# tmdt-buw/VQ-VAE-Transformer-Arc-Welding

Measured on AMD Instinct MI355X. Metric: welding windows/sec (train) VQ-VAE+8-blk Transformer at 1/2/4/8 MI355X, higher is better.
Workload: dtype bf16; 1 GPU; VQ-VAE-Patch reconstruction train step (configs[1]); global_batch=1024, per_gpu_batch=1024, seq_len=200, codebook=512x64, hidden=512, n_resblocks=8, patch=25, parallelism=dp1, optimizer=RAdam(lr 1e-3), operands=bf16 (opt-in), fp32 accumulation and master weights

## Files before the change

### include/arcweld_amd.h

```cpp
#ifndef ARCWELD_AMD_H
#define ARCWELD_AMD_H

#include <stdint.h>

#ifdef __cplusplus
extern "C" {
#endif

enum { AW_OK = 0, AW_ERR_ARG = -1, AW_ERR_LAUNCH = -2 };
enum { AW_F32 = 0, AW_BF16 = 1 };
enum { AW_ACT_GELU_ERF = 0, AW_ACT_GELU_TANH = 1, AW_ACT_DERIV = 2 };

const char* aw_last_error(void);
int aw_version(void);

typedef struct {
  int M, N, K;
  int a_dtype;
  const void* A; int64_t lda; int a_trans;
  const void* B; int64_t ldb; int b_trans;
  int conv_cin, conv_seg, conv_dir, conv_operand;
  float alpha, beta;
  const float* bias;
  int act;
// ... 62 lines not shown
  int head_k;
  const void* head_in;
  const void* head_w;
  const float* head_bias;
  void* head_patches;
  int head_L, head_C, head_P;
} aw_res_chain_fwd_args;
typedef struct {
  int64_t N;
  int H, R;
  int taps, seg;
  const void* gx;
  const void* gxo;
  const void* x0;
  const void* w1t[AW_RES_CHAIN_MAX];
  const void* w2t[AW_RES_CHAIN_MAX];
  const void* dgelu_h[AW_RES_CHAIN_MAX];
  const void* dgelu_x[AW_RES_CHAIN_MAX];
  void* gh[AW_RES_CHAIN_MAX];
  void* gxo_out[AW_RES_CHAIN_MAX];
  float drop_p;
  int store_policy;
  const uint64_t* drop_masks;
} aw_res_chain_bwd_args;
int aw_res_chain_fwd(const aw_res_chain_fwd_args* args, void* stream);
int aw_res_chain_bwd(const aw_res_chain_bwd_args* args, void* stream);
int64_t aw_res_dropout_masks_bytes(int64_t N, int R);
int aw_res_dropout_masks(int64_t N, int R, float drop_p, const uint64_t* drop_seed, const uint64_t* seed_ptr,
                         void* masks, void* stream);
#define AW_RES_PACK_MAX 32
int aw_res_pack_weights(const void* const* src, void* const* fwd, void* const* bwd, int n, int taps, void* stream);
int aw_res_pack_weights_mixed(const void* const* src, void* const* fwd, void* const* bwd, const int* job_taps, int n,
                              int taps, void* stream);

int aw_vq_forward(const float* z, const float* E, int64_t N, int K, int D,
                  float* zq, int64_t* idx, float* counts, double* sqerr, void* stream);
int aw_vq_forward_ex(const float* z, const float* E, int64_t N, int K, int D, float* zq, int64_t* idx, float* counts,
                     double* sqerr, void* zq_copy, int copy_dtype, void* stream);
#define AW_VQ_COUNT_GROUPS_MAX 64
int aw_vq_forward_ex2(const float* z, const float* E, int64_t N, int K, int D, float* zq, int64_t* idx, float* counts,
                      int count_groups, double* sqerr, void* zq_copy, int copy_dtype, void* stream);
int aw_vq_finalize(const float* counts, const double* sqerr, int64_t N, int K, int D, float beta,
                   float* loss, float* perplexity, void* stream);
int aw_vq_finalize_ex(const float* counts, int count_groups, const double* sqerr, int64_t N, int K, int D, float beta,
                      float* loss, float* perplexity, void* stream);
int aw_vq_backward(const float* z, const float* E, const int64_t* idx, const float* g_zq, const float* g_loss,
// ... 208 lines not shown
```

### vq-vae-transformer-arc-welding_amd/arcweld/_native.py

```python
from __future__ import annotations

import ctypes
import os

import torch

PKG_DIR = os.path.dirname(os.path.dirname(os.path.abspath(__file__)))
LIB_PATH = os.environ.get("ARCWELD_LIB") or os.path.join(PKG_DIR, "lib", "libarcweld_amd.so")
HEADER = os.path.join(os.path.dirname(PKG_DIR), "include", "arcweld_amd.h")

AW_F32, AW_BF16 = 0, 1
AW_ACT_GELU_ERF, AW_ACT_GELU_TANH, AW_ACT_DERIV = 0, 1, 2
AW_STORE_NT, AW_STORE_WT = 0, 1

c_i64 = ctypes.c_int64
c_int = ctypes.c_int
c_f = ctypes.c_float
c_p = ctypes.c_void_p


class GemmArgs(ctypes.Structure):
    _fields_ = [
        ("M", c_int), ("N", c_int), ("K", c_int),
        ("a_dtype", c_int),
# ... 36 lines not shown
RES_PACK_MAX = 32
RES_TAIL_MAX = 8
SAMPLE_MAX_V = 16384
_E = RES_CHAIN_MAX


class ResChainFwdArgs(ctypes.Structure):
    _fields_ = [("N", c_i64), ("H", c_int), ("R", c_int), ("taps", c_int), ("seg", c_int), ("a0", c_p), ("x0", c_p),
                ("w1", c_p * _E), ("w2", c_p * _E), ("b1", c_p * _E), ("b2", c_p * _E),
                ("dgelu_h", c_p * _E), ("a1", c_p * _E), ("dgelu_x", c_p * _E), ("a", c_p * _E),
                ("drop_p", c_f), ("drop_seed", ctypes.c_uint64 * _E), ("seed_ptr", c_p), ("store_policy", c_int),
                ("drop_masks", c_p),
                ("tail_k1", c_int), ("tail_w", c_p * RES_TAIL_MAX), ("tail_bias", c_p), ("tail_y", c_p),
                ("tail_colstats", c_p),
                ("sep_d", c_int), ("sep_w", c_p), ("sep_bias", c_p), ("sep_z", c_p),
                ("head_k", c_int), ("head_in", c_p), ("head_w", c_p), ("head_bias", c_p), ("head_patches", c_p),
                ("head_L", c_int), ("head_C", c_int), ("head_P", c_int)]


class ResChainBwdArgs(ctypes.Structure):
    _fields_ = [("N", c_i64), ("H", c_int), ("R", c_int), ("taps", c_int), ("seg", c_int), ("gx", c_p), ("gxo", c_p),
                ("x0", c_p), ("w1t", c_p * _E), ("w2t", c_p * _E), ("dgelu_h", c_p * _E), ("dgelu_x", c_p * _E),
                ("gh", c_p * _E), ("gxo_out", c_p * _E),
                ("drop_p", c_f), ("store_policy", c_int), ("drop_masks", c_p)]


class SampleArgs(ctypes.Structure):
    _fields_ = [("logits", c_p), ("B", c_int), ("V", c_int), ("n_valid", c_int),
                ("top_k", c_int), ("top_p", c_f), ("min_p", c_f), ("inv_temperature", c_f),
                ("do_sample", c_int), ("seed", ctypes.c_uint64), ("step", c_i64),
                ("ids_out", c_p), ("ld_ids", c_i64), ("col", c_i64),
                ("u_out", c_p),
                ("logp_out", c_p), ("logq_out", c_p), ("ld_lp", c_i64), ("col_lp", c_i64),
                ("n_kept_out", c_p), ("thr_out", c_p),
                ("bad_count", c_p)]


BEAM_MAX_W = 32


class BeamArgs(ctypes.Structure):
    _fields_ = [("logits", c_p), ("ldl", c_i64), ("B", c_int), ("W_in", c_int), ("W_out", c_int), ("V", c_int),
                ("n_valid", c_int),
                ("scores_in", c_p),
                ("scores_out", c_p), ("parent_out", c_p), ("token_out", c_p), ("logp_out", c_p),
                ("bad_count", c_p)]

# ... 181 lines not shown
```

### vq-vae-transformer-arc-welding_amd/arcweld/kernels.py

```python
from __future__ import annotations

import contextvars
import ctypes

import torch

from . import _native as nat
from ._native import AW_ACT_DERIV, AW_ACT_GELU_ERF, AW_ACT_GELU_TANH, AW_BF16, AW_F32, GemmArgs, call, dtype_code, ptr, stream_ptr

__all__ = ["gemm", "AW_ACT_DERIV", "AW_ACT_GELU_ERF", "AW_ACT_GELU_TANH", "AW_BF16", "AW_F32"]


def _ld(t):
    if t is None:
        return 0
    if t.dim() == 1:
        return t.shape[0]
    if t.stride(-1) != 1:
        raise nat.NativeError("operand rows must be contiguous (stride(-1) == 1)")
    return t.stride(0)


_STORE_POLICY = contextvars.ContextVar("arcweld_store_policy", default=0)

# ... 309 lines not shown
            hp = None
        else:
            hp, P = head[3], int(head[4])
            if hin.dtype != torch.float32 or hin.dim() != 3 or not hin.is_contiguous():
                raise nat.NativeError("res_chain_fwd: the encoder head's input must be contiguous (B, L, C) float32 windows")
            Bw, Lw, Cw = hin.shape
            if not (1 <= P <= hk) or (Lw * Cw) % P or Bw * (Lw * Cw // P) != N:
                raise nat.NativeError(f"res_chain_fwd: windows {tuple(hin.shape)} do not make {N} patches of {P}")
            if hp is not None and (hp.dtype != torch.bfloat16 or tuple(hp.shape) != (N, hk) or not hp.is_contiguous()):
                raise nat.NativeError(f"res_chain_fwd: patches must be a contiguous ({N}, {hk}) bfloat16 tensor")
            g.head_patches, g.head_L, g.head_C, g.head_P = ptr(hp), Lw, Cw, P
        g.head_k, g.head_in, g.head_w, g.head_bias = hk, ptr(hin), ptr(hw), ptr(hb)
        flops += 2.0 * N * H * (hk if taps == 3 else P)
        extra += [hin, hw, hb, hp]
    elif a0 is None or x0 is None:
        raise nat.NativeError("res_chain_fwd: a0 / x0 missing")
    _maybe_timed(stream, "gemm_bf16", flops,
                 lambda sp: call("aw_res_chain_fwd", ctypes.byref(g), sp),
                 lambda: (f"res_chain_fwd_kernel<{int(taps)}>",
                          _nbytes([a0, x0, masks] + list(w1) + list(w2) + list(b1) + list(b2) + list(dh) + list(a1) +
                                  list(dx)[:-1] + list(a) + extra)))


def res_chain_bwd(gx, gxo, w1t, w2t, dh, x0, dx, gh, gxo_out, drop_p=0.0, masks=None, taps=1, seg=16, stream=None):
    N, H = gx.shape
    R = len(w1t)
    if not (1 <= R <= RES_CHAIN_MAX) or not all(len(v) == R for v in (w2t, dh, dx, gh, gxo_out)):
        raise nat.NativeError("res_chain_bwd: need R (1..16) entries in every per-block list")
    _chk_rows([gx, gxo, x0] + list(dh) + list(dx[1:]) + list(gh) + list(gxo_out), N, H, "res_chain_bwd")
    g = nat.ResChainBwdArgs()
    g.N, g.H, g.R, g.taps, g.seg = N, H, R, int(taps), int(seg)
    g.gx, g.gxo, g.x0 = ptr(gx), ptr(gxo), ptr(x0)
    for r in range(R):
        g.w1t[r], g.w2t[r], g.dgelu_h[r] = ptr(w1t[r]), ptr(w2t[r]), ptr(dh[r])
        g.dgelu_x[r] = ptr(dx[r]) if r > 0 else None
        g.gh[r], g.gxo_out[r] = ptr(gh[r]), ptr(gxo_out[r])
    g.drop_p = float(drop_p)
    g.store_policy = _chain_store_policy()
    g.drop_masks = ptr(masks)
    _maybe_timed(stream, "gemm_bf16", _chain_flops(R, N, H, taps, seg),
                 lambda sp: call("aw_res_chain_bwd", ctypes.byref(g), sp),
                 lambda: (f"res_chain_bwd_kernel<{int(taps)}>",
                          _nbytes([gx, gxo, x0, masks] + list(w1t) + list(w2t) + list(dh) + list(dx[1:]) + list(gh) +
                                  list(gxo_out))))


def res_pack_weights(src, fwd=None, bwd=None, taps=1, stream=None, job_taps=None):
    n = len(src)
    fwd = fwd if fwd is not None else [None] * n
    bwd = bwd if bwd is not None else [None] * n
    jt = [int(taps)] * n if job_taps is None else [int(v) for v in job_taps]
    if len(fwd) != n or len(bwd) != n or len(jt) != n:
        raise nat.NativeError("res_pack_weights: list lengths differ")
    for i in range(n):
        for t in (src[i], fwd[i], bwd[i]):
            if t is not None and (t.dtype != torch.bfloat16 or t.numel() != 512 * 512 * jt[i] or not t.is_contiguous()):
                raise nat.NativeError(f"res_pack_weights: need contiguous 512 x {512 * jt[i]} bfloat16 tensors")
    for c0 in range(0, n, nat.RES_PACK_MAX):
        sl = slice(c0, c0 + nat.RES_PACK_MAX)
        m = len(src[sl])
        arr = lambda ts: (ctypes.c_void_p * m)(*[ptr(t) for t in ts])
        if job_taps is None:
            call("aw_res_pack_weights", arr(src[sl]), arr(fwd[sl]), arr(bwd[sl]), m, int(taps), stream_ptr(stream))
        else:
            call("aw_res_pack_weights_mixed", arr(src[sl]), arr(fwd[sl]), arr(bwd[sl]), (ctypes.c_int * m)(*jt[sl]), m,
                 int(taps), stream_ptr(stream))

# ... 659 lines not shown
```

### vq-vae-transformer-arc-welding_amd/arcweld/resstack.py

```python
from __future__ import annotations

import torch

from . import kernels as K

F32 = torch.float32


def _centre_job(w, out):
    O, I = w.shape[0], w.shape[1]
    c = w[:, :, 1]
    if w.is_contiguous():
        return (w, O, I, 3, 1, 0, out)
    if not c.is_contiguous():
        raise ValueError("encoder conv weight: unsupported layout")
    return (c, O, I, 1, 0, 0, out)


def _centre_grad(g):
    O, I = g.shape[0], g.shape[1]
    if g.is_contiguous():
        return g.view(O, 3 * I), (0, 3, 1)
    c = g[:, :, 1]
    if not c.is_contiguous():
# ... 117 lines not shown
    sv.xs += [e(RT) if save and r < R - 1 else None for r in range(R)]
    sv.a0s += [e(T) for _ in range(R)]
    wsrc = [w for r in range(R) for w in weights[r]]
    pk = [torch.empty(H, geo.Kd, device=dev, dtype=T) for _ in wsrc]
    ktail = None
    if tail is not None:
        Wt, tb, Y, cst = tail
        k1 = Wt.shape[0] // H
        tsrc = [Wt[j * H:(j + 1) * H] for j in range(k1)]
        tpk = [torch.empty(H, H, device=dev, dtype=T) for _ in tsrc]
        K.res_pack_weights(wsrc + tsrc, pk + tpk, None, taps=taps, job_taps=[taps] * len(wsrc) + [1] * k1)
        ktail = (tpk, tb, Y, cst)
    else:
        K.res_pack_weights(wsrc, pk, None, taps=taps)
    if save:
        sv.pk_bwd = wsrc
        if sv.p_drop > 0 and R > 1:
            sv.masks = K.res_dropout_masks_empty(N, R, dev)
    K.res_chain_fwd(a0, x0, pk[0::2], pk[1::2], [b1 for b1, _ in biases], [b2 for _, b2 in biases], sv.hs, sv.a1s,
                    sv.xs[1:], sv.a0s[1:], drop=(sv.p_drop, sv.seeds), seed_ptr=sv.ctr, masks=sv.masks, taps=taps,
                    seg=geo.S, tail=ktail, sep=sep, head=head)


def _chain_bwd(sv, gx, gxo, grads):
    N, H = gx.shape
    geo = sv.geo
    R, taps, dev, T = len(sv.hs), geo.taps, gx.device, gxo.dtype
    gh = [torch.empty(N, H, device=dev, dtype=T) for _ in range(R)]
    go = [torch.empty(N, H, device=dev, dtype=T) for _ in range(R)]
    pk_bwd = [torch.empty(H, geo.Kd, device=dev, dtype=T) for _ in sv.pk_bwd]
    K.res_pack_weights(sv.pk_bwd, None, pk_bwd, taps=taps)
    K.res_chain_bwd(gx, gxo, pk_bwd[0::2], pk_bwd[1::2], sv.hs, sv.xs[0], [None] + list(sv.xs[1:R]), gh, go,
                    drop_p=sv.p_drop, masks=sv.masks, taps=taps, seg=geo.S)
    sv.pk_bwd = sv.masks = None
    wgrads = []
    for r in reversed(range(R)):
        gin = gxo if r == R - 1 else go[r + 1]
        wgrads.append(geo.wgrad_problem(gin, sv.a1s[r], *grads(r, 1)))
        wgrads.append(geo.wgrad_problem(gh[r], sv.a0s[r], *grads(r, 0)))
    return go[0], wgrads


def forward(geo, x0, a0, weights, biases, bns=None, *, T, RT, p_drop=0.0, seeds=None, ctr=None, training=False,
            chain=False, last_operand_only=True, in_place=False, save=True, tail=None, sep=None, head=None):
    R, H, Kd = len(biases), geo.H, geo.Kd
    N, dev = a0.shape[0], a0.device
    seeds = [0] * R if seeds is None else seeds
    route = "bn" if bns is not None else "chain" if chain else "conv"
    sv = Saved(geo, route, T, p_drop, seeds, ctr, training, x0, a0)
    e = lambda dt: torch.empty(N, H, device=dev, dtype=dt)
    if tail is not None and (route != "chain" or geo.taps != 3):
        raise ValueError("resstack.forward: the ConvT tail runs only inside the decoder chain")
    if sep is not None and (route != "chain" or geo.taps != 1):
        raise ValueError("resstack.forward: the sep tail runs only inside the encoder chain")
    if head is not None and route != "chain":
        raise ValueError("resstack.forward: a head runs only inside a chain launch")
# ... 6 lines not shown
        last = last_operand_only and r == R - 1
        if route == "bn":
            xn, an, bs = _bn_block_fwd(geo, a, x, w1, w2, b1, b2, bns[r], training, p_drop, seeds[r], ctr, T, last)
        else:
            if h is None or not in_place:
                h, a1 = e(T), e(T)
            K.gemm(a, w1, N, H, Kd, bias=b1, C=h, C2=a1, c2_mode=1, **geo.fwd)
            xn = None if last else x if in_place else e(RT)
            an = a if in_place else e(T)
            out = dict(C=an) if last else dict(C=xn, C2=an, c2_mode=1)
            K.gemm(a1, w2, N, H, Kd, bias=b2, drop=(p_drop, seeds[r]), seed_ptr=ctr, resid=x, **out, **geo.fwd)
            bs = None
        if save:
            sv.xs.append(xn)
            sv.a0s.append(an)
            sv.hs.append(h)
            sv.a1s.append(a1)
            sv.bs.append(bs)
            sv.ws.append((w1, w2))
        x, a = xn, an
    return x, a, sv


def backward(sv, gy, go, dweights, grads, bns=None, slot=None, r0_copy=True):
    if sv.route == "chain":
        gxo, wgrads = _chain_bwd(sv, gy, go, grads)
        return gxo, gxo, wgrads
    N, H = gy.shape
    geo, RT, T, p = sv.geo, gy.dtype, sv.T, sv.p_drop
    e = lambda dt: torch.empty(N, H, device=gy.device, dtype=dt)
    wgrads = []
    for r in reversed(range(len(sv.hs))):
        W1d, W2d = dweights[r]
        if sv.route == "bn":
            gy, go = _bn_block_bwd(sv, r, gy, W1d, W2d, grads, bns[r], slot, wgrads, r0_copy and r == 0)
            continue
        gh = e(T)
        K.gemm(go, W2d, N, H, geo.Kd, b_trans=True, pre=sv.hs[r], C=gh, **geo.dgrad)
        wgrads.append(geo.wgrad_problem(go, sv.a1s[r], *grads(r, 1)))
        gyn = e(RT)
        gon = e(T) if r > 0 or r0_copy else None
        K.gemm(gh, W1d, N, H, geo.Kd, b_trans=True, pre=sv.xs[r], resid=gy, C=gyn, C2=gon,
               c2_mode=3 if r > 0 else 2 if r0_copy else 0, drop2=(p, sv.seeds[r - 1] if r > 0 else 0),
               seed_ptr=sv.ctr, **geo.dgrad)
        wgrads.append(geo.wgrad_problem(gh, sv.a0s[r], *grads(r, 0)))
        gy, go = gyn, gon
    return gy, go, wgrads
```

### vq-vae-transformer-arc-welding_amd/arcweld/vqvae.py

```python
from __future__ import annotations

import os
import weakref

import torch

from . import _native as nat
from . import kernels as K
from . import operands
from . import resstack
from .precision import operand_dtype

F32 = torch.float32


def _mix(seed: int, salt: int) -> int:
    z = (seed * 0x9E3779B97F4A7C15 + salt * 0xBF58476D1CE4E5B9 + 0x94D049BB133111EB) & 0xFFFFFFFFFFFFFFFF
    z ^= z >> 31
    z = (z * 0xD6E8FEB86659FD93) & 0xFFFFFFFFFFFFFFFF
    return z ^ (z >> 32)


def rng_snapshot(m, dev, p_drop, zero=None):
    if p_drop <= 0.0:
# ... 59 lines not shown
    pass


def _operand_jobs(m, T):
    from .operands import OperandJob as J
    sh = VQVAEShapes(m, 1)
    H, D, R, P, k1 = sh.H, sh.D, sh.R, sh.P, sh.k1
    pr = _params(m)
    dev = pr["pe"].weight.device
    e = lambda *s: torch.empty(*s, device=dev, dtype=T)
    jobs = [J("Wp", pr["pe"].weight, H, 1, P, 0, 4, torch.zeros(H, sh.ldp, device=dev, dtype=T),
              sh.ldp)]
    centre = lambda w: resstack._centre_job(w, None)[:6]
    for r, (c1, c2) in enumerate(pr["enc"]):
        for nm, c in (("1", c1), ("2", c2)):
            jobs.append(J(f"enc{r}_{nm}", c.weight, H, H, 1, 0, 0, e(H, H), derive=centre))
    jobs.append(J("Ws", pr["sep"].weight, D, H, 1, 0, 0, e(D, H)))
    jobs.append(J("Wd0", pr["dec0"].weight, H, D, 1, 0, 0, e(H, D)))
    for r, (c1, c2) in enumerate(pr["dec"]):
        for nm, c in (("1", c1), ("2", c2)):
            jobs.append(J(f"dec{r}_{nm}", c.weight, H, H, 3, 0, 1, e(H, 3 * H)))
            jobs.append(J(f"dgw{r}_{nm}", c.weight, H, H, 3, 0, 2, e(3 * H, H)))
    jobs.append(J("Wt1", pr["t1"].weight, H, H, k1, 0, 3, e(k1 * H, H)))
    return jobs


def operand_set(m, T=None):
    T = operand_dtype(T)
    return operands.peek(m, ("vqvae", T), lambda: _operand_jobs(m, T))


@K.store_policy(nat.AW_STORE_WT)
def forward(m, x, training: bool, need_backward: bool, dtype=None, seed: int = 0, head=True):
    T = operand_dtype(dtype)
    if x.dtype != F32 or x.dim() != 3:
        raise ValueError("VQVAEPatch expects float32 windows of shape (B, seq_len, input_dim)")
    x = x.contiguous()
    sh = VQVAEShapes(m, x.shape[0])
    H, D, N, S, R, P, k1 = sh.H, sh.D, sh.N, sh.S, sh.R, sh.P, sh.k1
    if x.shape[1] != sh.L or x.shape[2] != sh.C:
        raise ValueError(f"expected windows (B, {sh.L}, {sh.C}), got {tuple(x.shape)}")
    pr = _params(m)
    dev = x.device
    p_drop = float(m.dropout_p) if training else 0.0
    e = lambda *s, dt=F32: torch.empty(*s, device=dev, dtype=dt)
    sv = Saved()
    sv.sh, sv.T, sv.p_drop, sv.training = sh, T, p_drop, training
# ... 237 lines not shown
    g_xhat = g_xhat.contiguous()
    bn = pr["bn"]

    gsums = sv.head_gsums
    owner = m.__dict__.get("_acc_owner")
    if owner is not None and owner() is sv:
        m.__dict__["_acc_owner"] = None
    if not getattr(sv, "head_pass1_done", False):
        K.unpatch_head_bwd1(sv.Y2, sh.Q, sv.stats, pr["t2"].weight.view(H, 5), g_xhat, gsums,
                            slot(pr["t2"].weight).view(H, 5), slot(pr["t2"].bias), slot(bn.weight), slot(bn.bias))
    gY = e(N * k1, H, dt=T)
    K.unpatch_head_bwd2(sv.Y2, sh.Q, sv.stats, pr["t2"].weight.view(H, 5), g_xhat, gsums, sv.training, gY,
                        slot(pr["t1"].bias))
    gY2 = gY.view(N, k1 * H)
    K.gemm(sv.yR_T, gY2, H, k1 * H, N, a_trans=True, b_trans=True, C=slot(pr["t1"].weight).view(H, H * k1),
           accumulate=True, col_map=(H, k1, 0))
    RT = sv.RT
    gy, go = e(N, H, dt=RT), e(N, H, dt=T)
    bnm = m.batch_norm and R > 0
    K.gemm(gY2, sv.Wt1, N, H, k1 * H, b_trans=True, C=gy, C2=None if bnm else go, c2_mode=0 if bnm else
           (3 if R > 0 else 2), drop2=(p_drop, sv.dec.seeds[-1] if R > 0 else 0), seed_ptr=sv.ctr)

    dgw = [(sv.ops[f"dgw{r}_1"], sv.ops[f"dgw{r}_2"]) for r in range(R)]
    gy, go, wgrads = resstack.backward(sv.dec, gy, go, dgw, _grads(pr["dec"], slot), pr["dec_bn"], slot)
    K.gemm_grouped(wgrads)

    K.gemm(go, sv.zq_T, H, D, N, a_trans=True, b_trans=True, C=slot(pr["dec0"].weight).view(H, D), accumulate=True,
           a_rowsum=slot(pr["dec0"].bias))
    gzq = e(N, D)
    K.gemm(go, sv.Wd0, N, D, H, b_trans=True, C=gzq)

    dz = e(N, D)
    dz_T = dz if T == F32 else None
    if pr["E"] is None:
        res, qs = sv.rvq
        nq = res.shape[0]
        K.rvq_backward(res, qs, gzq, g_emb if nq == 1 else g_emb.expand(nq).contiguous(), dz)
    else:
        dz_T = dz if T == F32 else e(N, D, dt=T)
        K.vq_backward(sv.z, pr["E"], sv.idx, gzq, g_emb, m.vector_quantization.beta, dz, slot(pr["E"]),
                      dz_copy=None if T == F32 else dz_T)
    if mid_hook is not None:
        with K.store_policy(nat.AW_STORE_NT):
            mid_hook()
    if dz_T is None:
        dz_T = _cast(dz, T)

    K.gemm(dz_T, sv.xR_T, D, H, N, a_trans=True, b_trans=True, C=slot(pr["sep"].weight).view(D, H), accumulate=True,
           a_rowsum=slot(pr["sep"].bias))
    gx, gxo = e(N, H, dt=RT), e(N, H, dt=T)
    K.gemm(dz_T, sv.Ws, N, H, D, b_trans=True, C=gx, C2=None if bnm else gxo, c2_mode=0 if bnm else
           (3 if R > 0 else 2), drop2=(p_drop, sv.enc.seeds[-1] if R > 0 else 0), seed_ptr=sv.ctr)

    gx, gxo, wgrads = resstack.backward(sv.enc, gx, gxo, sv.enc.ws, _grads(pr["enc"], slot), pr["enc_bn"], slot)
    K.wgrad_issue(wgrads)

    K.gemm(gxo, sv.patches, H, P, N, a_trans=True, b_trans=True, C=slot(pr["pe"].weight).view(H, P),
           accumulate=True, a_rowsum=slot(pr["pe"].bias))


class VQVAEPatchFunction(torch.autograd.Function):

    @staticmethod
    def forward(ctx, m, x, seed, *params):
        training = m.training
        need = torch.is_grad_enabled() or any(p.requires_grad for p in params)
        emb, x_hat, perp, idx, sv = forward(m, x, training, need_backward=True, seed=seed)
        ctx.m, ctx.sv, ctx.params = m, sv, params
        if perp is not None:
            ctx.mark_non_differentiable(perp)
        m._last_indices = idx
        return emb, x_hat, perp

    @staticmethod
    def backward(ctx, g_emb, g_xhat, g_perp):
        m, sv = ctx.m, ctx.sv
        sink = getattr(m, "_grad_sink", None)
# ... 19 lines not shown
```

### vq-vae-transformer-arc-welding_amd/csrc/reschain.hip

```cpp
#include "common.h"

#include <type_traits>

#pragma clang diagnostic ignored "-Winline-asm"


namespace {

constexpr int EC_H = 512;
constexpr int EC_ROWS = 64;
constexpr int EC_NTH = 512;
constexpr int EC_ROWB = EC_H * 2;
constexpr int EC_SCR = 2048;
constexpr int EC_SEG = 16;

template <int TAPS> struct EcGeo {
  static constexpr int KS = 16 * TAPS;
  static constexpr int JS = (TAPS == 1 ? 16 : 17) * EC_ROWB;
  static constexpr int R0 = TAPS == 1 ? 0 : EC_ROWB;
  static constexpr int IMG = (TAPS == 1 ? 64 : 69) * EC_ROWB;
  static constexpr int SCR = 2 * IMG;
  static constexpr int FLAGS = SCR + 8 * EC_SCR;
  static constexpr int BIAS = FLAGS + 64;
  static constexpr int LDS = BIAS + 8 * 256;
// ... 576 lines not shown
    for (int e = 0; e < 4; ++e) bv[e] = P.sep_bias[16 * i + 4 * L.g + e];
    f32x4 acc[2] = {f32x4{0.f, 0.f, 0.f, 0.f}, f32x4{0.f, 0.f, 0.f, 0.f}};
#pragma unroll
    for (int s = 0; s < 16; ++s) {
      if ((s & 1) == 0 && (s >> 1) != L.w) ec_wait<G>(smem, s >> 1, NC);
#pragma unroll
      for (int jj = 0; jj < 2; ++jj) {
        const uint4 bf = ec_lds_r16(smem, (L.rb[0] ^ (64 * (s & 3))) + (s >> 2) * 256 + (j0 + jj) * G::JS);
        acc[jj] = __builtin_amdgcn_mfma_f32_16x16x32_bf16(__builtin_bit_cast(bf16x8, ws[s]),
                                                          __builtin_bit_cast(bf16x8, bf), acc[jj], 0, 0, 0);
      }
    }
    const rsrc_t rz = ec_rsrc(P.sep_z, (uint32_t)(P.N * 64 * 4));
#pragma unroll
    for (int jj = 0; jj < 2; ++jj) {
      uint4 v;
      v.x = __float_as_uint(acc[jj][0] + bv[0]), v.y = __float_as_uint(acc[jj][1] + bv[1]);
      v.z = __float_as_uint(acc[jj][2] + bv[2]), v.w = __float_as_uint(acc[jj][3] + bv[3]);
      ec_store16<WT>(rz, (uint32_t)(((row0 + 16 * (j0 + jj) + L.li) * 64 + 16 * i + 4 * L.g) * 4), 0, v);
    }
  }
}

template <int TAPS, bool DROP, bool WT>
__global__ __launch_bounds__(EC_NTH) void res_chain_bwd_kernel(aw_res_chain_bwd_args P) {
  using G = EcGeo<TAPS>;
  __shared__ __attribute__((aligned(16))) char smem[G::LDS];
  const int tid = threadIdx.x;
  const int64_t row0 = (int64_t)blockIdx.x * EC_ROWS;
  const EcLane<G, -1> L(tid);
  const uint32_t nbytes = (uint32_t)(P.N * EC_ROWB);
  const int R = P.R, NC = 2 * R;
  const uint32_t fo = ec_frag_off(row0, L.li, L.w, L.g);

  ec_init<G>(smem, tid);
  ec_load_image<G>(smem, P.gxo, row0, nbytes, tid);
  u32x2 gr[4][4];
  ec_load_frags(gr, ec_rsrc(P.gx, nbytes), fo);
  uint4 wf[2][4];
  {
    const rsrc_t r0 = ec_rsrc(P.w2t[R - 1], G::WBYTES);
#pragma unroll
    for (int i = 0; i < 4; ++i) {
      wf[0][i] = ec_wload(r0, L.wl, ec_woff<G>(i, 0));
      wf[1][i] = ec_wload(r0, L.wl, ec_woff<G>(i, 1));
    }
  }
  asm volatile("s_waitcnt lgkmcnt(0)" ::: "memory");
  __syncthreads();

  for (int c = 0; c < NC; ++c) {
    const int r = R - 1 - (c >> 1);
    const bool second = (c & 1) != 0;
    const rsrc_t rc = ec_rsrc(second ? P.w1t[r] : P.w2t[r], G::WBYTES);
    const bool has_next = c + 1 < NC;
    const rsrc_t rn = ec_rsrc(has_next ? (second ? P.w2t[r - 1] : P.w1t[r]) : nullptr, G::WBYTES);
    const int io = (c & 1) * G::IMG, no = ((c + 1) & 1) * G::IMG;
    f32x4 acc[4][4];
    uint4 pl[8];
    u32x2 keep = {0u, 0u};
    auto load_pre = [&] {
      const rsrc_t rp = ec_rsrc(second ? (r > 0 ? P.dgelu_x[r] : P.x0) : P.dgelu_h[r], nbytes);
      const uint32_t gs = (uint32_t)(((row0 + (L.lane >> 3)) * EC_H + 64 * L.w + 8 * (L.lane & 7)) * 2);
#pragma unroll
      for (int q = 0; q < 8; ++q) {
        const auto v = __builtin_amdgcn_raw_buffer_load_b128(rp, gs, 8192 * q, 0);
        memcpy(&pl[q], &v, 16);
      }
      if (DROP && second && r > 0) keep = ec_keep(P.drop_masks, r - 1, tid);
    };
    ec_conv<G>(acc, wf, smem, L.rb, io, rc, rn, has_next, L.wl, L.w, c, load_pre, [](int) {});
    int nwb[4];
// ... 46 lines not shown
          for (int i = 0; i < 4; ++i) {
            float v[4], ds[4] = {1.f, 1.f, 1.f, 1.f}, o[4];
            grad(i, j, v, std::false_type{});
            if constexpr (DROP) ec_scales(keep, i, j, dk, ds);
#pragma unroll
            for (int e = 0; e < 4; ++e) o[e] = v[e] * ds[e];
            ec_lds_w8(smem, nwb[i] + G::JS * j, ec_pack(o));
            ec_frag_fence(4 * j + i);
          }
        }
        ec_publish<G>(smem, L.w, L.lane, c + 1);
      } else {
#pragma unroll
        for (int j = 0; j < 4; ++j) {
          stage_pre(j);
#pragma unroll
          for (int i = 0; i < 4; ++i) {
            float v[4];
            grad(i, j, v, std::true_type{});
            ec_lds_w8(smem, nwb[i] + G::JS * j, gr[i][j]);
            ec_frag_fence(4 * j + i);
          }
        }
      }
      ec_store_slice<G, WT>(smem, no, S, ec_rsrc(P.gxo_out[r], nbytes));
    }
  }
}

struct PackJobs {
  const void* src[AW_RES_PACK_MAX];
  void* fwd[AW_RES_PACK_MAX];
  void* bwd[AW_RES_PACK_MAX];
  uint32_t one_tap;
};

constexpr int PK_PITCH1 = 128 + 16;
template <int TAPS>
__device__ __forceinline__ void res_pack_fwd(const char* __restrict__ W, uint4* __restrict__ out, char* t, int x,
                                             int nx, int tid) {
  constexpr int RB = EC_ROWB * TAPS, PITCH0 = RB + 16, KB = 16 * TAPS;
  for (int mb = x; mb < EC_H / 16; mb += nx) {
#pragma unroll
    for (int q = 0; q < 4 * TAPS; ++q) {
      const int c = tid + 256 * q, row = c / (64 * TAPS), kc = c % (64 * TAPS);
      *reinterpret_cast<uint4*>(t + row * PITCH0 + kc * 16) =
          *reinterpret_cast<const uint4*>(W + (size_t)(16 * mb + row) * RB + kc * 16);
    }
// ... 48 lines not shown
  uint64_t seed[AW_RES_CHAIN_MAX];
};
__global__ __launch_bounds__(EC_NTH) void res_mask_kernel(MaskSeeds S, const uint64_t* seed_ptr, uint32_t thr,
                                                          u32x2* __restrict__ out) {
  const int tid = threadIdx.x, r = blockIdx.y;
  const int lane = tid & 63, w = tid >> 6, g = lane >> 4, li = lane & 15;
  const uint64_t seed = aw_seed_mix(S.seed[r], seed_ptr);
  const uint64_t grp0 = (((uint64_t)blockIdx.x * EC_ROWS + li) * EC_H >> 2) + 16 * w + g;
  uint32_t k[2] = {0u, 0u};
#pragma unroll
  for (int f = 0; f < 16; ++f) k[f >> 3] |= ec_keep_bits(seed, grp0, f, thr);
  out[((size_t)r * gridDim.x + blockIdx.x) * EC_NTH + tid] = u32x2{k[0], k[1]};
}

bool aligned16(const void* p) { return ((uintptr_t)p & 15) == 0; }

template <int TAPS, bool TAIL, bool HEAD>
void launch_fwd(const aw_res_chain_fwd_args* a, bool drop, bool wt, dim3 grid, hipStream_t s) {
  if (drop && wt) hipLaunchKernelGGL((res_chain_fwd_kernel<TAPS, true, true, TAIL, HEAD>), grid, dim3(EC_NTH), 0, s, *a);
  else if (drop) hipLaunchKernelGGL((res_chain_fwd_kernel<TAPS, true, false, TAIL, HEAD>), grid, dim3(EC_NTH), 0, s, *a);
  else if (wt) hipLaunchKernelGGL((res_chain_fwd_kernel<TAPS, false, true, TAIL, HEAD>), grid, dim3(EC_NTH), 0, s, *a);
  else hipLaunchKernelGGL((res_chain_fwd_kernel<TAPS, false, false, TAIL, HEAD>), grid, dim3(EC_NTH), 0, s, *a);
}
template <int TAPS>
void launch_bwd(const aw_res_chain_bwd_args* a, bool drop, bool wt, dim3 grid, hipStream_t s) {
  if (drop && wt) hipLaunchKernelGGL((res_chain_bwd_kernel<TAPS, true, true>), grid, dim3(EC_NTH), 0, s, *a);
  else if (drop) hipLaunchKernelGGL((res_chain_bwd_kernel<TAPS, true, false>), grid, dim3(EC_NTH), 0, s, *a);
  else if (wt) hipLaunchKernelGGL((res_chain_bwd_kernel<TAPS, false, true>), grid, dim3(EC_NTH), 0, s, *a);
  else hipLaunchKernelGGL((res_chain_bwd_kernel<TAPS, false, false>), grid, dim3(EC_NTH), 0, s, *a);
}

}

#define CHAIN_SHAPE_CHECKS(who)                                                                                       \
  AW_REQUIRE(a, who ": null args");                                                                                   \
  AW_REQUIRE(a->H == EC_H, who ": H must be %d (got %d)", EC_H, a->H);                                                \
  AW_REQUIRE(a->R >= 1 && a->R <= AW_RES_CHAIN_MAX, who ": R must be 1..%d", AW_RES_CHAIN_MAX);                       \
  AW_REQUIRE(a->N >= 1 && (a->N + EC_ROWS) * EC_ROWB < (1ll << 31), who ": N out of range");                          \
  AW_REQUIRE(a->taps == 1 || (a->taps == 3 && a->seg == EC_SEG && a->N % EC_SEG == 0),                                \
             who ": taps must be 1, or 3 with seg == %d and N %% %d == 0 (taps %d, seg %d)", EC_SEG, EC_SEG, a->taps, \
             a->seg);                                                                                                 \
  AW_REQUIRE(a->drop_p >= 0.f && a->drop_p < 1.f, who ": drop_p out of [0, 1)")

extern "C" int aw_res_chain_fwd(const aw_res_chain_fwd_args* a, void* stream) {
  CHAIN_SHAPE_CHECKS("aw_res_chain_fwd");
  if (a->head_k == 0) {
    AW_REQUIRE(!a->head_in && !a->head_w && !a->head_bias && !a->head_patches && !a->head_L && !a->head_C && !a->head_P,
               "aw_res_chain_fwd: head fields without head_k");
    AW_REQUIRE(a->a0 && a->x0, "aw_res_chain_fwd: a0 / x0 missing");
  } else {
    AW_REQUIRE(a->head_k == (a->taps == 3 ? 64 : 32), "aw_res_chain_fwd: head_k must be 64 (taps 3) or 32 (taps 1), got %d",
               a->head_k);
// ... 35 lines not shown
  const dim3 grid((unsigned)((a->N + EC_ROWS - 1) / EC_ROWS));
  const bool drop = a->drop_p > 0.f, wt = a->store_policy == AW_STORE_WT;
  if (a->sep_d == 0) {
    AW_REQUIRE(!a->sep_w && !a->sep_bias && !a->sep_z, "aw_res_chain_fwd: sep fields without sep_d");
  } else {
    AW_REQUIRE(a->taps == 1 && a->sep_d == 64, "aw_res_chain_fwd: the sep tail needs taps == 1 and sep_d == 64 (got %d)",
               a->sep_d);
    AW_REQUIRE(a->sep_w && aligned16(a->sep_w) && a->sep_bias && a->sep_z && aligned16(a->sep_z),
               "aw_res_chain_fwd: sep_w / sep_bias / sep_z missing or unaligned");
  }
  const bool head = a->head_k != 0;
  if (a->taps == 3) {
    if (a->tail_k1) head ? launch_fwd<3, true, true>(a, drop, wt, grid, s) : launch_fwd<3, true, false>(a, drop, wt, grid, s);
    else head ? launch_fwd<3, false, true>(a, drop, wt, grid, s) : launch_fwd<3, false, false>(a, drop, wt, grid, s);
  } else {
    if (a->sep_d) head ? launch_fwd<1, true, true>(a, drop, wt, grid, s) : launch_fwd<1, true, false>(a, drop, wt, grid, s);
    else head ? launch_fwd<1, false, true>(a, drop, wt, grid, s) : launch_fwd<1, false, false>(a, drop, wt, grid, s);
  }
  return aw::check_launch("aw_res_chain_fwd");
}

extern "C" int aw_res_chain_bwd(const aw_res_chain_bwd_args* a, void* stream) {
  CHAIN_SHAPE_CHECKS("aw_res_chain_bwd");
  AW_REQUIRE(a->gx && a->gxo && a->x0 && aligned16(a->gx) && aligned16(a->gxo) && aligned16(a->x0),
             "aw_res_chain_bwd: gx / gxo / x0 missing or unaligned");
  for (int r = 0; r < a->R; ++r) {
    AW_REQUIRE(a->w1t[r] && a->w2t[r] && aligned16(a->w1t[r]) && aligned16(a->w2t[r]),
               "aw_res_chain_bwd: block %d weights missing or unaligned", r);
    AW_REQUIRE(a->dgelu_h[r] && aligned16(a->dgelu_h[r]) && (r == 0 || (a->dgelu_x[r] && aligned16(a->dgelu_x[r]))),
               "aw_res_chain_bwd: block %d saved GELU' missing or unaligned", r);
    AW_REQUIRE(a->gh[r] && a->gxo_out[r] && aligned16(a->gh[r]) && aligned16(a->gxo_out[r]),
               "aw_res_chain_bwd: block %d outputs missing or unaligned", r);
  }
  AW_REQUIRE(a->drop_p == 0.f || a->R == 1 || (a->drop_masks && aligned16(a->drop_masks)),
             "aw_res_chain_bwd: drop_p > 0 needs drop_masks");
  hipStream_t s = (hipStream_t)stream;
  const dim3 grid((unsigned)((a->N + EC_ROWS - 1) / EC_ROWS));
  const bool drop = a->drop_p > 0.f && a->R > 1, wt = a->store_policy == AW_STORE_WT;
  if (a->taps == 3) launch_bwd<3>(a, drop, wt, grid, s);
  else launch_bwd<1>(a, drop, wt, grid, s);
  return aw::check_launch("aw_res_chain_bwd");
}

extern "C" int aw_res_pack_weights(const void* const* src, void* const* fwd, void* const* bwd, int n, int taps,
                                   void* stream) {
  return aw_res_pack_weights_mixed(src, fwd, bwd, nullptr, n, taps, stream);
}

extern "C" int aw_res_pack_weights_mixed(const void* const* src, void* const* fwd, void* const* bwd,
                                         const int* job_taps, int n, int taps, void* stream) {
  AW_REQUIRE(src && fwd && bwd && n >= 0 && n <= AW_RES_PACK_MAX && (taps == 1 || taps == 3),
             "aw_res_pack_weights: bad args (n must be 0..%d, taps 1 or 3)", AW_RES_PACK_MAX);
  if (n == 0) return AW_OK;
  PackJobs J{};
  for (int i = 0; i < n; ++i) {
    AW_REQUIRE(src[i] && aligned16(src[i]) && aligned16(fwd[i]) && aligned16(bwd[i]) && (fwd[i] || bwd[i]) &&
                   src[i] != fwd[i] && src[i] != bwd[i], "aw_res_pack_weights: job %d: missing, aliased or unaligned", i);
    J.src[i] = src[i];
    J.fwd[i] = fwd[i];
    J.bwd[i] = bwd[i];
    if (job_taps && job_taps[i] != taps) {
      AW_REQUIRE(job_taps[i] == 1 && fwd[i] && !bwd[i], "aw_res_pack_weights: job %d: a job of %d taps in a launch of "
                 "%d (only 1-tap forward copies may differ)", i, job_taps[i], taps);
// ... 25 lines not shown
```

Measured before the change: 442,800 windows/s.

## Fuse sep-gradient head and dec0 gradient tail into residual chain backward kernel

Moves the dz·Ws gradient GEMM (with dropout scaling) into the prologue of the encoder residual-chain backward kernel, and the go·Wd0 gradient GEMM into the epilogue of the decoder chain backward kernel. This removes two separate GEMM launches along with the global round-trips of gx/go, and the data stays in LDS/registers instead. Both paths need extra pre-transposed bf16 weight copies packed per step, and the extra registers and LDS publishing could lower occupancy or add sync in the chain kernel. The fused kernels are on by default and can be disabled through environment variables.

```diff
diff --git a/include/arcweld_amd.h b/include/arcweld_amd.h
--- a/include/arcweld_amd.h
+++ b/include/arcweld_amd.h
@@ -108,6 +108,15 @@
   float drop_p;
   int store_policy;
   const uint64_t* drop_masks;
+  int tail_d;
+  const void* tail_w;
+  float* tail_gzq;
+  int head_k;
+  const void* head_in;
+  const void* head_w;
+  void* head_gxo;
+  uint64_t head_drop_seed;
+  const uint64_t* seed_ptr;
 } aw_res_chain_bwd_args;
 int aw_res_chain_fwd(const aw_res_chain_fwd_args* args, void* stream);
 int aw_res_chain_bwd(const aw_res_chain_bwd_args* args, void* stream);
diff --git a/vq-vae-transformer-arc-welding_amd/arcweld/_native.py b/vq-vae-transformer-arc-welding_amd/arcweld/_native.py
--- a/vq-vae-transformer-arc-welding_amd/arcweld/_native.py
+++ b/vq-vae-transformer-arc-welding_amd/arcweld/_native.py
@@ -82,7 +82,10 @@
     _fields_ = [("N", c_i64), ("H", c_int), ("R", c_int), ("taps", c_int), ("seg", c_int), ("gx", c_p), ("gxo", c_p),
                 ("x0", c_p), ("w1t", c_p * _E), ("w2t", c_p * _E), ("dgelu_h", c_p * _E), ("dgelu_x", c_p * _E),
                 ("gh", c_p * _E), ("gxo_out", c_p * _E),
-                ("drop_p", c_f), ("store_policy", c_int), ("drop_masks", c_p)]
+                ("drop_p", c_f), ("store_policy", c_int), ("drop_masks", c_p),
+                ("tail_d", c_int), ("tail_w", c_p), ("tail_gzq", c_p),
+                ("head_k", c_int), ("head_in", c_p), ("head_w", c_p), ("head_gxo", c_p),
+                ("head_drop_seed", ctypes.c_uint64), ("seed_ptr", c_p)]
 
 
 class SampleArgs(ctypes.Structure):
diff --git a/vq-vae-transformer-arc-welding_amd/arcweld/kernels.py b/vq-vae-transformer-arc-welding_amd/arcweld/kernels.py
--- a/vq-vae-transformer-arc-welding_amd/arcweld/kernels.py
+++ b/vq-vae-transformer-arc-welding_amd/arcweld/kernels.py
@@ -355,8 +355,19 @@
                                   list(dx)[:-1] + list(a) + extra)))
 
 
-def res_chain_bwd(gx, gxo, w1t, w2t, dh, x0, dx, gh, gxo_out, drop_p=0.0, masks=None, taps=1, seg=16, stream=None):
-    N, H = gx.shape
+def bwd_tail_ok():
+    import os
+    return os.environ.get("ARCWELD_BWD_TAIL", "1") != "0"
+
+
+def bwd_head_ok():
+    import os
+    return os.environ.get("ARCWELD_BWD_HEAD", "1") != "0"
+
+
+def res_chain_bwd(gx, gxo, w1t, w2t, dh, x0, dx, gh, gxo_out, drop_p=0.0, masks=None, taps=1, seg=16, stream=None,
+                  head=None, tail=None):
+    N, H = gxo.shape
     R = len(w1t)
     if not (1 <= R <= RES_CHAIN_MAX) or not all(len(v) == R for v in (w2t, dh, dx, gh, gxo_out)):
         raise nat.NativeError("res_chain_bwd: need R (1..16) entries in every per-block list")
@@ -371,11 +382,41 @@
     g.drop_p = float(drop_p)
     g.store_policy = _chain_store_policy()
     g.drop_masks = ptr(masks)
-    _maybe_timed(stream, "gemm_bf16", _chain_flops(R, N, H, taps, seg),
+    flops, extra, D = _chain_flops(R, N, H, taps, seg), [], 64
+    if tail is not None:
+        wt, gzq = tail
+        if taps != 3:
+            raise nat.NativeError("res_chain_bwd: the tail needs taps == 3")
+        if wt.dtype != torch.bfloat16 or tuple(wt.shape) != (D, H) or not wt.is_contiguous():
+            raise nat.NativeError(f"res_chain_bwd: tail weights must be a contiguous ({D}, {H}) bfloat16 copy")
+        if gzq.dtype != torch.float32 or tuple(gzq.shape) != (N, D) or not gzq.is_contiguous():
+            raise nat.NativeError(f"res_chain_bwd: tail gzq must be a contiguous ({N}, {D}) float32 tensor")
+        g.tail_d, g.tail_w, g.tail_gzq = D, ptr(wt), ptr(gzq)
+        flops += 2.0 * N * D * H
+        extra += [wt, gzq]
+    if head is not None:
+        dz, wt, seed, seed_ptr = head
+        if taps != 1:
+            raise nat.NativeError("res_chain_bwd: the head needs taps == 1")
+        if gx is not None:
+            raise nat.NativeError("res_chain_bwd: with a head gx is made in the launch (pass None)")
+        if dz.dtype != torch.bfloat16 or tuple(dz.shape) != (N, D) or not dz.is_contiguous():
+            raise nat.NativeError(f"res_chain_bwd: the head's input must be a contiguous ({N}, {D}) bfloat16 tensor")
+        if wt.dtype != torch.bfloat16 or tuple(wt.shape) != (H, D) or not wt.is_contiguous():
+            raise nat.NativeError(f"res_chain_bwd: head weights must be a contiguous ({H}, {D}) bfloat16 copy")
+        g.gxo, g.head_gxo = None, ptr(gxo)
+        g.head_k, g.head_in, g.head_w = D, ptr(dz), ptr(wt)
+        if drop_p > 0 and masks is None:
+            g.head_drop_seed, g.seed_ptr = int(seed) & 0xFFFFFFFFFFFFFFFF, ptr(seed_ptr)
+        flops += 2.0 * N * H * D
+        extra += [dz, wt]
+    elif gx is None:
+        raise nat.NativeError("res_chain_bwd: gx missing")
+    _maybe_timed(stream, "gemm_bf16", flops,
                  lambda sp: call("aw_res_chain_bwd", ctypes.byref(g), sp),
                  lambda: (f"res_chain_bwd_kernel<{int(taps)}>",
                           _nbytes([gx, gxo, x0, masks] + list(w1t) + list(w2t) + list(dh) + list(dx[1:]) + list(gh) +
-                                  list(gxo_out))))
+                                  list(gxo_out) + extra)))
 
 
 def res_pack_weights(src, fwd=None, bwd=None, taps=1, stream=None, job_taps=None):
diff --git a/vq-vae-transformer-arc-welding_amd/arcweld/resstack.py b/vq-vae-transformer-arc-welding_amd/arcweld/resstack.py
--- a/vq-vae-transformer-arc-welding_amd/arcweld/resstack.py
+++ b/vq-vae-transformer-arc-welding_amd/arcweld/resstack.py
@@ -163,16 +163,18 @@
                     seg=geo.S, tail=ktail, sep=sep, head=head)
 
 
-def _chain_bwd(sv, gx, gxo, grads):
-    N, H = gx.shape
+def _chain_bwd(sv, gx, gxo, grads, head=None, tail=None):
+    N, H = gxo.shape
     geo = sv.geo
-    R, taps, dev, T = len(sv.hs), geo.taps, gx.device, gxo.dtype
+    R, taps, dev, T = len(sv.hs), geo.taps, gxo.device, gxo.dtype
+    if head is not None:
+        head = (head[0], head[1], sv.seeds[-1], sv.ctr)
     gh = [torch.empty(N, H, device=dev, dtype=T) for _ in range(R)]
     go = [torch.empty(N, H, device=dev, dtype=T) for _ in range(R)]
     pk_bwd = [torch.empty(H, geo.Kd, device=dev, dtype=T) for _ in sv.pk_bwd]
     K.res_pack_weights(sv.pk_bwd, None, pk_bwd, taps=taps)
     K.res_chain_bwd(gx, gxo, pk_bwd[0::2], pk_bwd[1::2], sv.hs, sv.xs[0], [None] + list(sv.xs[1:R]), gh, go,
-                    drop_p=sv.p_drop, masks=sv.masks, taps=taps, seg=geo.S)
+                    drop_p=sv.p_drop, masks=sv.masks, taps=taps, seg=geo.S, head=head, tail=tail)
     sv.pk_bwd = sv.masks = None
     wgrads = []
     for r in reversed(range(R)):
@@ -225,9 +227,13 @@
     return x, a, sv
 
 
-def backward(sv, gy, go, dweights, grads, bns=None, slot=None, r0_copy=True):
+def backward(sv, gy, go, dweights, grads, bns=None, slot=None, r0_copy=True, head=None, tail=None):
+    if head is not None and (sv.route != "chain" or sv.geo.taps != 1):
+        raise ValueError("resstack.backward: the sep gradient head runs only inside the encoder chain")
+    if tail is not None and (sv.route != "chain" or sv.geo.taps != 3):
+        raise ValueError("resstack.backward: the 1x1 gradient tail runs only inside the decoder chain")
     if sv.route == "chain":
-        gxo, wgrads = _chain_bwd(sv, gy, go, grads)
+        gxo, wgrads = _chain_bwd(sv, gy, go, grads, head, tail)
         return gxo, gxo, wgrads
     N, H = gy.shape
     geo, RT, T, p = sv.geo, gy.dtype, sv.T, sv.p_drop
diff --git a/vq-vae-transformer-arc-welding_amd/arcweld/vqvae.py b/vq-vae-transformer-arc-welding_amd/arcweld/vqvae.py
--- a/vq-vae-transformer-arc-welding_amd/arcweld/vqvae.py
+++ b/vq-vae-transformer-arc-welding_amd/arcweld/vqvae.py
@@ -105,7 +105,17 @@
             jobs.append(J(f"dec{r}_{nm}", c.weight, H, H, 3, 0, 1, e(H, 3 * H)))
             jobs.append(J(f"dgw{r}_{nm}", c.weight, H, H, 3, 0, 2, e(3 * H, H)))
     jobs.append(J("Wt1", pr["t1"].weight, H, H, k1, 0, 3, e(k1 * H, H)))
+    RT = resid_dtype(m, T)
+    if _bwd_bounds_shape(H, D, T) and K.res_chain_ok(H, R, T, RT) and pr["enc_bn"] is None and K.bwd_head_ok():
+        jobs.append(J("WsT", pr["sep"].weight, H, D, 1, 0, 3, e(H, D)))
+    if (_bwd_bounds_shape(H, D, T) and K.res_chain_ok(H, R, T, RT, 3, sh.S, "DEC") and pr["dec_bn"] is None
+            and K.bwd_tail_ok()):
+        jobs.append(J("Wd0T", pr["dec0"].weight, D, H, 1, 0, 3, e(D, H)))
     return jobs
+
+
+def _bwd_bounds_shape(H, D, T):
+    return T == torch.bfloat16 and H == 512 and D == 64
 
 
 def operand_set(m, T=None):
@@ -389,13 +399,16 @@
            (3 if R > 0 else 2), drop2=(p_drop, sv.dec.seeds[-1] if R > 0 else 0), seed_ptr=sv.ctr)
 
     dgw = [(sv.ops[f"dgw{r}_1"], sv.ops[f"dgw{r}_2"]) for r in range(R)]
-    gy, go, wgrads = resstack.backward(sv.dec, gy, go, dgw, _grads(pr["dec"], slot), pr["dec_bn"], slot)
+    gzq = e(N, D)
+    bwd_tail = sv.dec.route == "chain" and "Wd0T" in sv.ops and K.bwd_tail_ok()
+    gy, go, wgrads = resstack.backward(sv.dec, gy, go, dgw, _grads(pr["dec"], slot), pr["dec_bn"], slot,
+                                       tail=(sv.ops["Wd0T"], gzq) if bwd_tail else None)
     K.gemm_grouped(wgrads)
 
     K.gemm(go, sv.zq_T, H, D, N, a_trans=True, b_trans=True, C=slot(pr["dec0"].weight).view(H, D), accumulate=True,
            a_rowsum=slot(pr["dec0"].bias))
-    gzq = e(N, D)
-    K.gemm(go, sv.Wd0, N, D, H, b_trans=True, C=gzq)
+    if not bwd_tail:
+        K.gemm(go, sv.Wd0, N, D, H, b_trans=True, C=gzq)
 
     dz = e(N, D)
     dz_T = dz if T == F32 else None
@@ -415,11 +428,14 @@
 
     K.gemm(dz_T, sv.xR_T, D, H, N, a_trans=True, b_trans=True, C=slot(pr["sep"].weight).view(D, H), accumulate=True,
            a_rowsum=slot(pr["sep"].bias))
-    gx, gxo = e(N, H, dt=RT), e(N, H, dt=T)
-    K.gemm(dz_T, sv.Ws, N, H, D, b_trans=True, C=gx, C2=None if bnm else gxo, c2_mode=0 if bnm else
-           (3 if R > 0 else 2), drop2=(p_drop, sv.enc.seeds[-1] if R > 0 else 0), seed_ptr=sv.ctr)
-
-    gx, gxo, wgrads = resstack.backward(sv.enc, gx, gxo, sv.enc.ws, _grads(pr["enc"], slot), pr["enc_bn"], slot)
+    bwd_head = sv.enc.route == "chain" and "WsT" in sv.ops and K.bwd_head_ok()
+    gx, gxo = None if bwd_head else e(N, H, dt=RT), e(N, H, dt=T)
+    if not bwd_head:
+        K.gemm(dz_T, sv.Ws, N, H, D, b_trans=True, C=gx, C2=None if bnm else gxo, c2_mode=0 if bnm else
+               (3 if R > 0 else 2), drop2=(p_drop, sv.enc.seeds[-1] if R > 0 else 0), seed_ptr=sv.ctr)
+
+    gx, gxo, wgrads = resstack.backward(sv.enc, gx, gxo, sv.enc.ws, _grads(pr["enc"], slot), pr["enc_bn"], slot,
+                                        head=(dz_T, sv.ops["WsT"]) if bwd_head else None)
     K.wgrad_issue(wgrads)
 
     K.gemm(gxo, sv.patches, H, P, N, a_trans=True, b_trans=True, C=slot(pr["pe"].weight).view(H, P),
diff --git a/vq-vae-transformer-arc-welding_amd/csrc/reschain.hip b/vq-vae-transformer-arc-welding_amd/csrc/reschain.hip
--- a/vq-vae-transformer-arc-welding_amd/csrc/reschain.hip
+++ b/vq-vae-transformer-arc-welding_amd/csrc/reschain.hip
@@ -622,9 +622,10 @@
   }
 }
 
-template <int TAPS, bool DROP, bool WT>
+template <int TAPS, bool DROP, bool WT, bool TAIL, bool HEAD>
 __global__ __launch_bounds__(EC_NTH) void res_chain_bwd_kernel(aw_res_chain_bwd_args P) {
   using G = EcGeo<TAPS>;
+  static_assert((!TAIL || TAPS == 3) && (!HEAD || TAPS == 1), "the decoder's tail, the encoder's head");
   __shared__ __attribute__((aligned(16))) char smem[G::LDS];
   const int tid = threadIdx.x;
   const int64_t row0 = (int64_t)blockIdx.x * EC_ROWS;
@@ -634,20 +635,91 @@
   const uint32_t fo = ec_frag_off(row0, L.li, L.w, L.g);
 
   ec_init<G>(smem, tid);
-  ec_load_image<G>(smem, P.gxo, row0, nbytes, tid);
   u32x2 gr[4][4];
-  ec_load_frags(gr, ec_rsrc(P.gx, nbytes), fo);
   uint4 wf[2][4];
-  {
+  u32x2 hkeep = {0u, 0u};
+  if constexpr (!HEAD) {
+    ec_load_image<G>(smem, P.gxo, row0, nbytes, tid);
+    ec_load_frags(gr, ec_rsrc(P.gx, nbytes), fo);
     const rsrc_t r0 = ec_rsrc(P.w2t[R - 1], G::WBYTES);
 #pragma unroll
     for (int i = 0; i < 4; ++i) {
       wf[0][i] = ec_wload(r0, L.wl, ec_woff<G>(i, 0));
       wf[1][i] = ec_wload(r0, L.wl, ec_woff<G>(i, 1));
     }
+  } else {
+    const int tok = tid >> 3, pc = tid & 7;
+    const auto v = __builtin_amdgcn_raw_buffer_load_b128(ec_rsrc(P.head_in, (uint32_t)(P.N * 128)),
+                                                         (uint32_t)((row0 + tok) * 128 + pc * 16), 0, 0);
+    uint4 u;
+    memcpy(&u, &v, 16);
+    *reinterpret_cast<uint4*>(smem + G::IMG + ec_off<G>(tok, pc)) = u;
+    const rsrc_t rh = ec_rsrc(P.head_w, EC_H * 128);
+    const int ho = (64 * L.w + L.li) * 128 + 16 * L.g;
+#pragma unroll
+    for (int i = 0; i < 4; ++i)
+#pragma unroll
+      for (int s = 0; s < 2; ++s) wf[s][i] = ec_wload(rh, ho, i * 16 * 128 + 64 * s);
+    if constexpr (DROP) {
+      if (P.drop_masks) {
+        hkeep = ec_keep(P.drop_masks, R - 1, tid);
+      } else {
+        const uint64_t seed = aw_seed_mix(P.head_drop_seed, P.seed_ptr);
+        const uint64_t grp0 = (uint64_t)(row0 + L.li) * (EC_H / 4) + 16 * L.w + L.g;
+        const uint32_t thr = aw_drop_threshold(P.drop_p);
+        uint32_t kb[2] = {0u, 0u};
+#pragma unroll
+        for (int f = 0; f < 16; ++f) kb[f >> 3] |= ec_keep_bits(seed, grp0, f, thr);
+        hkeep = u32x2{kb[0], kb[1]};
+      }
+    }
   }
   asm volatile("s_waitcnt lgkmcnt(0)" ::: "memory");
   __syncthreads();
+
+  if constexpr (HEAD) {
+    f32x4 acc[4][4];
+#pragma unroll
+    for (int i = 0; i < 4; ++i)
+#pragma unroll
+      for (int j = 0; j < 4; ++j) acc[i][j] = f32x4{0.f, 0.f, 0.f, 0.f};
+    const rsrc_t r0 = ec_rsrc(P.w2t[R - 1], G::WBYTES);
+    const int rbi = L.rb[0] + G::IMG;
+#pragma unroll
+    for (int s = 0; s < 2; ++s) {
+      uint4 bf[4];
+#pragma unroll
+      for (int j = 0; j < 4; ++j) bf[j] = ec_lds_r16(smem, (rbi ^ (64 * s)) + j * G::JS);
+#pragma unroll
+      for (int i = 0; i < 4; ++i)
+#pragma unroll
+        for (int j = 0; j < 4; ++j)
+          acc[i][j] = __builtin_amdgcn_mfma_f32_16x16x32_bf16(__builtin_bit_cast(bf16x8, wf[s][i]),
+                                                              __builtin_bit_cast(bf16x8, bf[j]), acc[i][j], 0, 0, 0);
+#pragma unroll
+      for (int i = 0; i < 4; ++i) wf[s][i] = ec_wload(r0, L.wl, ec_woff<G>(i, s));
+      __builtin_amdgcn_sched_barrier(0);
+    }
+    const float dk = DROP ? 1.f / (1.f - P.drop_p) : 1.f;
+#pragma unroll
+    for (int j = 0; j < 4; ++j)
+#pragma unroll
+      for (int i = 0; i < 4; ++i) {
+        float v[4], ds[4] = {1.f, 1.f, 1.f, 1.f}, o[4];
+#pragma unroll
+        for (int e = 0; e < 4; ++e) v[e] = acc[i][j][e];
+        gr[i][j] = ec_pack(v);
+        if constexpr (DROP) ec_scales(hkeep, i, j, dk, ds);
+#pragma unroll
+        for (int e = 0; e < 4; ++e) o[e] = v[e] * ds[e];
+        ec_lds_w8(smem, L.wb(i) + G::JS * j, DROP ? ec_pack(o) : gr[i][j]);
+        ec_frag_fence(4 * j + i);
+      }
+    asm volatile("s_waitcnt lgkmcnt(0)" ::: "memory");
+    __syncthreads();
+    const EcStore<G> S(tid, row0);
+    ec_store_slice<G, WT>(smem, 0, S, ec_rsrc(P.head_gxo, nbytes));
+  }
 
   for (int c = 0; c < NC; ++c) {
     const int r = R - 1 - (c >> 1);
@@ -740,8 +812,39 @@
             ec_frag_fence(4 * j + i);
           }
         }
+        if constexpr (TAIL) ec_publish<G>(smem, L.w, L.lane, c + 1);
       }
       ec_store_slice<G, WT>(smem, no, S, ec_rsrc(P.gxo_out[r], nbytes));
+    }
+  }
+
+  if constexpr (TAIL) {
+    constexpr int TC = G::KS / 32;
+    __builtin_amdgcn_sched_barrier(0);
+    const int i = L.w & 3, j0 = 2 * (L.w >> 2);
+    const rsrc_t rw = ec_rsrc(P.tail_w, 64 * EC_ROWB);
+    const int wo = (16 * i + L.li) * EC_ROWB + 16 * L.g;
+    uint4 ws[16];
+#pragma unroll
+    for (int s = 0; s < 16; ++s) ws[s] = ec_wload(rw, wo, 64 * s);
+    f32x4 acc[2] = {f32x4{0.f, 0.f, 0.f, 0.f}, f32x4{0.f, 0.f, 0.f, 0.f}};
+#pragma unroll
+    for (int s = 0; s < 16; ++s) {
+      if ((s & 1) == 0 && (s >> 1) != L.w) ec_wait<G>(smem, s >> 1, NC);
+#pragma unroll
+      for (int jj = 0; jj < 2; ++jj) {
+        const uint4 bf = ec_lds_r16(smem, (L.rb[TC] ^ (64 * (s & 3))) + (s >> 2) * 256 + (j0 + jj) * G::JS);
+        acc[jj] = __builtin_amdgcn_mfma_f32_16x16x32_bf16(__builtin_bit_cast(bf16x8, ws[s]),
+                                                          __builtin_bit_cast(bf16x8, bf), acc[jj], 0, 0, 0);
+      }
+    }
+    const rsrc_t rz = ec_rsrc(P.tail_gzq, (uint32_t)(P.N * 64 * 4));
+#pragma unroll
+    for (int jj = 0; jj < 2; ++jj) {
+      uint4 v;
+      v.x = __float_as_uint(acc[jj][0]), v.y = __float_as_uint(acc[jj][1]);
+      v.z = __float_as_uint(acc[jj][2]), v.w = __float_as_uint(acc[jj][3]);
+      ec_store16<WT>(rz, (uint32_t)(((row0 + 16 * (j0 + jj) + L.li) * 64 + 16 * i + 4 * L.g) * 4), 0, v);
     }
   }
 }
@@ -836,12 +939,12 @@
   else if (wt) hipLaunchKernelGGL((res_chain_fwd_kernel<TAPS, false, true, TAIL, HEAD>), grid, dim3(EC_NTH), 0, s, *a);
   else hipLaunchKernelGGL((res_chain_fwd_kernel<TAPS, false, false, TAIL, HEAD>), grid, dim3(EC_NTH), 0, s, *a);
 }
-template <int TAPS>
+template <int TAPS, bool TAIL, bool HEAD>
 void launch_bwd(const aw_res_chain_bwd_args* a, bool drop, bool wt, dim3 grid, hipStream_t s) {
-  if (drop && wt) hipLaunchKernelGGL((res_chain_bwd_kernel<TAPS, true, true>), grid, dim3(EC_NTH), 0, s, *a);
-  else if (drop) hipLaunchKernelGGL((res_chain_bwd_kernel<TAPS, true, false>), grid, dim3(EC_NTH), 0, s, *a);
-  else if (wt) hipLaunchKernelGGL((res_chain_bwd_kernel<TAPS, false, true>), grid, dim3(EC_NTH), 0, s, *a);
-  else hipLaunchKernelGGL((res_chain_bwd_kernel<TAPS, false, false>), grid, dim3(EC_NTH), 0, s, *a);
+  if (drop && wt) hipLaunchKernelGGL((res_chain_bwd_kernel<TAPS, true, true, TAIL, HEAD>), grid, dim3(EC_NTH), 0, s, *a);
+  else if (drop) hipLaunchKernelGGL((res_chain_bwd_kernel<TAPS, true, false, TAIL, HEAD>), grid, dim3(EC_NTH), 0, s, *a);
+  else if (wt) hipLaunchKernelGGL((res_chain_bwd_kernel<TAPS, false, true, TAIL, HEAD>), grid, dim3(EC_NTH), 0, s, *a);
+  else hipLaunchKernelGGL((res_chain_bwd_kernel<TAPS, false, false, TAIL, HEAD>), grid, dim3(EC_NTH), 0, s, *a);
 }
 
 }
@@ -923,8 +1026,27 @@
 
 extern "C" int aw_res_chain_bwd(const aw_res_chain_bwd_args* a, void* stream) {
   CHAIN_SHAPE_CHECKS("aw_res_chain_bwd");
-  AW_REQUIRE(a->gx && a->gxo && a->x0 && aligned16(a->gx) && aligned16(a->gxo) && aligned16(a->x0),
-             "aw_res_chain_bwd: gx / gxo / x0 missing or unaligned");
+  if (a->head_k == 0) {
+    AW_REQUIRE(!a->head_in && !a->head_w && !a->head_gxo && !a->head_drop_seed && !a->seed_ptr,
+               "aw_res_chain_bwd: head fields without head_k");
+    AW_REQUIRE(a->gx && a->gxo, "aw_res_chain_bwd: gx / gxo missing");
+  } else {
+    AW_REQUIRE(a->taps == 1 && a->head_k == 64, "aw_res_chain_bwd: the head needs taps == 1 and head_k == 64 (got %d)",
+               a->head_k);
+    AW_REQUIRE(!a->gx && !a->gxo, "aw_res_chain_bwd: with a head gx / gxo are made in the launch (pass NULL)");
+    AW_REQUIRE(a->head_in && a->head_w && a->head_gxo && aligned16(a->head_in) && aligned16(a->head_w) &&
+                   aligned16(a->head_gxo), "aw_res_chain_bwd: head_in / head_w / head_gxo missing or unaligned");
+  }
+  if (a->tail_d == 0) {
+    AW_REQUIRE(!a->tail_w && !a->tail_gzq, "aw_res_chain_bwd: tail fields without tail_d");
+  } else {
+    AW_REQUIRE(a->taps == 3 && a->tail_d == 64, "aw_res_chain_bwd: the tail needs taps == 3 and tail_d == 64 (got %d)",
+               a->tail_d);
+    AW_REQUIRE(a->tail_w && a->tail_gzq && aligned16(a->tail_w) && aligned16(a->tail_gzq),
+               "aw_res_chain_bwd: tail_w / tail_gzq missing or unaligned");
+  }
+  AW_REQUIRE(a->x0 && aligned16(a->gx) && aligned16(a->gxo) && aligned16(a->x0),
+             "aw_res_chain_bwd: x0 missing, or gx / gxo / x0 unaligned");
   for (int r = 0; r < a->R; ++r) {
     AW_REQUIRE(a->w1t[r] && a->w2t[r] && aligned16(a->w1t[r]) && aligned16(a->w2t[r]),
                "aw_res_chain_bwd: block %d weights missing or unaligned", r);
@@ -937,9 +1059,14 @@
              "aw_res_chain_bwd: drop_p > 0 needs drop_masks");
   hipStream_t s = (hipStream_t)stream;
   const dim3 grid((unsigned)((a->N + EC_ROWS - 1) / EC_ROWS));
-  const bool drop = a->drop_p > 0.f && a->R > 1, wt = a->store_policy == AW_STORE_WT;
-  if (a->taps == 3) launch_bwd<3>(a, drop, wt, grid, s);
-  else launch_bwd<1>(a, drop, wt, grid, s);
+  const bool drop = a->drop_p > 0.f && (a->R > 1 || a->head_k), wt = a->store_policy == AW_STORE_WT;
+  if (a->taps == 3) {
+    if (a->tail_d) launch_bwd<3, true, false>(a, drop, wt, grid, s);
+    else launch_bwd<3, false, false>(a, drop, wt, grid, s);
+  } else {
+    if (a->head_k) launch_bwd<1, false, true>(a, drop, wt, grid, s);
+    else launch_bwd<1, false, false>(a, drop, wt, grid, s);
+  }
   return aw::check_launch("aw_res_chain_bwd");
 }
 
```

After: 439,400 windows/s. About the same (-0.8%).
